# CHEBSB/PolarDecoding

Measured on AMD Instinct MI355X. Metric: decoded frames/sec, N=1024 K=512 CA-SCL L=8, higher is better.
Workload: dtype f64

## Files before the change

polardecoding_amd/csrc/scl_fast2.h:

```cpp
#pragma once
#include "octet_bits.h"
#include "scl_fast.h"

namespace polar {

template <typename R>
struct Fast2Cfg {
    static constexpr int NLOG = 10, N = 1024, NW = 32, TOP = 9, HI = 8, L = 8;
    static constexpr int NA = 32;
    static constexpr int WAVES = 4;
    static constexpr int MIN_WAVES_PER_SIMD = sizeof(R) == 8 ? 3 : 4;
    static constexpr int NFA = HI - 3;
    static constexpr size_t sc_l8 = 0;
    static constexpr size_t sc_l7 = sc_l8 + 8 * 256;
    static constexpr size_t sc_l6 = sc_l7 + 8 * 128;
    static constexpr size_t sc_tl = sc_l6 + 8 * 64;
    static constexpr size_t scratch_cw = sc_tl + 512;
    static constexpr size_t scratch_elems = 2 * scratch_cw;
    static constexpr size_t off_lut = 0;
    static constexpr size_t off_frz = off_lut + ((Lut<R>::bytes + 15) / 16) * 16;
    static constexpr size_t off_msk = off_frz + 4 * NW;
    static constexpr size_t off_kth = off_msk + 4 * CRC_MASK_ROWS * NW;
    static constexpr size_t off_stair = off_kth + 256 * 8;
    static constexpr size_t shared_bytes = off_stair + ((Stair<R>::bytes + 15) / 16) * 16;
    static constexpr size_t off_bl = 0;
    static constexpr size_t off_cw = off_bl + 4 * 2 * 8 * NW;
    static constexpr size_t off_cd = off_cw + 4 * 2 * 8 * NW;
    static constexpr size_t off_ky = off_cd + sizeof(R) * 32;
    static constexpr size_t off_sg = off_ky + 128;
    static constexpr size_t per_wave = off_sg + sizeof(R) * 512;
    static constexpr size_t total = shared_bytes + WAVES * per_wave;
};

template <int QP>
__device__ __forceinline__ double quadp(double x) { return quad_lanes<QP>(x); }
template <int QP>
__device__ __forceinline__ float quadp(float x) { return quad_lanes<QP>(x); }

template <bool FROM_Y>
struct Fast2Sigma { double sigma; };
template <>
struct Fast2Sigma<false> {};

template <typename R, typename IN, bool CRC_ON, bool FROM_Y>
struct Fast2Dec : Fast2Sigma<FROM_Y> {
    using C = Fast2Cfg<R>;
    static constexpr int N = C::N, NW = C::NW, TOP = C::TOP, HI = C::HI, L = 8, NFA = C::NFA;

    R A[C::NA];
    R a1;
    R bp_s, bp_d, bp_ts, bp_td;
    R PM;
    uint32_t ptr, bl0, fl;
    int logact;
    int p, c, pos, lane, gl;
    int own_addr, oth_addr;
    uint32_t pos0_mask;
    int cand_addr;
    Lut<R> lut;
    R *cand, *stg;
    uint32_t *blw, *curw, *keys;
    const unsigned char *kth;
    __amdgpu_buffer_rsrc_t rs_scr;
    __amdgpu_buffer_rsrc_t rs_in;
    unsigned cscr;
    unsigned csrc;
    static __device__ __forceinline__ __amdgpu_buffer_rsrc_t make_rsrc(const void *base, unsigned bytes)
    {
        return __builtin_amdgcn_make_buffer_rsrc(const_cast<void *>(base), 0, (int)bytes, 0x00020000);
    }
    typedef unsigned u2_t __attribute__((ext_vector_type(2)));
    static __device__ __forceinline__ double ld_buf(__amdgpu_buffer_rsrc_t r, unsigned eoff, double, int aux)
    {
        return aux ? __builtin_bit_cast(double, __builtin_amdgcn_raw_buffer_load_b64(r, eoff * 8u, 0, 16))
                   : __builtin_bit_cast(double, __builtin_amdgcn_raw_buffer_load_b64(r, eoff * 8u, 0, 0));
    }
    static __device__ __forceinline__ float ld_buf(__amdgpu_buffer_rsrc_t r, unsigned eoff, float, int aux)
    {
        return aux ? __builtin_bit_cast(float, __builtin_amdgcn_raw_buffer_load_b32(r, eoff * 4u, 0, 16))
                   : __builtin_bit_cast(float, __builtin_amdgcn_raw_buffer_load_b32(r, eoff * 4u, 0, 0));
    }
    static __device__ __forceinline__ void st_buf(__amdgpu_buffer_rsrc_t r, unsigned eoff, double v)
    {
        __builtin_amdgcn_raw_buffer_store_b64(__builtin_bit_cast(u2_t, v), r, eoff * 8u, 0, 0);
    }
    static __device__ __forceinline__ void st_buf(__amdgpu_buffer_rsrc_t r, unsigned eoff, float v)
    {
        __builtin_amdgcn_raw_buffer_store_b32(__builtin_bit_cast(unsigned, v), r, eoff * 4u, 0, 0);
    }
    struct SPtr {
        const Fast2Dec *d;
        unsigned off;
        struct Ref {
            const Fast2Dec *d;
            unsigned off;
            __device__ __forceinline__ void operator=(R v) const { st_buf(d->rs_scr, off, v); }
        };
        __device__ __forceinline__ SPtr operator+(int k) const { return SPtr{d, off + (unsigned)k}; }
        __device__ __forceinline__ Ref operator[](int k) const { return Ref{d, off + (unsigned)k}; }
    };
    static __device__ __forceinline__ R ld_sc(SPtr q) { return ld_buf(q.d->rs_scr, q.off, R(0), 1); }

    __device__ __forceinline__ int pa(int t) const { return (ptr >> (3 * (t - 4))) & 7; }
    __device__ __forceinline__ void set_pa(int t, int v) { ptr = (ptr & ~(7u << (3 * (t - 4)))) | ((uint32_t)v << (3 * (t - 4))); }
    __device__ __forceinline__ int pb(int t) const { return (ptr >> (3 * (NFA + t - 5))) & 7; }
    __device__ __forceinline__ void set_pb(int t, int v) { ptr = (ptr & ~(7u << (3 * (NFA + t - 5)))) | ((uint32_t)v << (3 * (NFA + t - 5))); }
    __device__ __forceinline__ R chk(R a, R b) const { return chk_lut1<R>(a, b, lut); }
    __device__ __forceinline__ R chks(R a, R b) const { return chk_lut1<R>(a, b, lut); }
    __device__ __forceinline__ R chv(int e) const
    {
        double v = (double)ld_buf(rs_in, csrc + (unsigned)e, IN(0), 0);
        if constexpr (FROM_Y) v = llr_from_y(v, this->sigma);
        return (R)v;
    }
    static __device__ __forceinline__ unsigned fresh(unsigned off)
    {
        __asm__ volatile("" : "+v"(off));
        return off;
    }
    __device__ __forceinline__ SPtr l8(int slot) const { return SPtr{this, fresh(cscr + (unsigned)(C::sc_l8 + slot * 256))}; }
    __device__ __forceinline__ SPtr l7(int slot) const { return SPtr{this, fresh(cscr + (unsigned)(C::sc_l7 + slot * 128))}; }
    __device__ __forceinline__ SPtr tls() const { return SPtr{this, fresh(cscr + (unsigned)C::sc_tl)}; }

    template <int T>
    __device__ __forceinline__ void f_reg()
    {
        constexpr int RO = (1 << T) / 4;
#pragma unroll
        for (int r = 0; r < RO; ++r) A[RO + r] = chk(A[2 * RO + r], A[3 * RO + r]);
        if constexpr (T >= 4) set_pa(T, p);
    }
    template <int T>
    __device__ __forceinline__ void g_reg()
    {
        constexpr int RO = (1 << T) / 4;
        const int sl = pa(T + 1) * 8 + gl;
        uint32_t w;
        if constexpr (T == 5) w = blw[pb(5) * NW + 1] >> pos;
        else w = bl0 >> (16 + pos);
#pragma unroll
        for (int r = 0; r < RO; ++r) {
            const R x = __shfl(A[2 * RO + r], sl), y = __shfl(A[3 * RO + r], sl);
            A[RO + r] = g_bit<R>(x, y, w, 4 * r);
        }
        set_pa(T, p);
    }
    __device__ __forceinline__ void g3()
    {
        const int sl = pa(4) * 8 + gl;
        const uint32_t w = bl0 >> (8 + pos);
#pragma unroll
        for (int r = 0; r < 2; ++r) {
            const R x = __shfl(A[4 + r], sl), y = __shfl(A[6 + r], sl);
            A[2 + r] = g_bit<R>(x, y, w, 4 * r);
        }
    }

    __device__ __forceinline__ void push_l6(R v)
    {
#pragma unroll
        for (int r = 16; r < 31; ++r) A[r] = A[r + 1];
        A[31] = v;
    }
    __device__ __forceinline__ void load_l6() { set_pa(6, p); }
    __device__ __forceinline__ R top_src(bool right, int idx, int q) const
    {
        const int seg = idx >> 4, within = idx & 15;
        const int e = 16 * q + within + 64 * (seg & 3) + 256 * (seg >> 2);
        return right ? chv(e) : ld_sc(tls() + e);
    }
    __device__ __forceinline__ void from_top(bool right, bool gstep)
    {
        vm_drain();
        const uint32_t *bt = blw + pb(TOP) * NW + 16;
        const uint32_t *bh = blw + pb(HI) * NW + 8;
        const SPtr o8 = l8(p), o7 = l7(p);
        const int w32 = (int)fresh((unsigned)(p * 4 + pos));
        const int nld = right ? 8 : 4;
        R *pre = A + 4;
#pragma unroll
        for (int m = 0; m < 8; ++m) pre[m] = (m < nld) ? top_src(right, w32 + 32 * m, 0) : R(0);
        for (int q = 0; q < 4; ++q) {
            lds_fence();
#pragma unroll
            for (int m = 0; m < 8; ++m)
                if (m < nld) stg[w32 + 32 * m] = pre[m];
            lds_fence();
            if (q < 3) {
#pragma unroll
                for (int m = 0; m < 8; ++m) pre[m] = (m < nld) ? top_src(right, w32 + 32 * m, q + 1) : R(0);
            }
#pragma unroll 1
            for (int i = 0; i < 4; ++i) {
                const int rr = 4 * q + i;
                const int e0 = pos + 4 * rr;
                const int sh = 4 * (rr & 7);
                const int wq = rr >> 3;
                const int wi = 4 * i + pos;
                R *v8 = A + 12;
#pragma unroll
                for (int k = 0; k < 4; ++k) {
                    const int e = e0 + 64 * k;
                    R x, y;
                    if (right) {
                        const uint32_t w0 = bt[2 * k + wq] >> pos, w1 = bt[8 + 2 * k + wq] >> pos;
                        x = g_bit<R>(stg[(k + 0) * 16 + wi], stg[(k + 8) * 16 + wi], w0, sh);
                        y = g_bit<R>(stg[(k + 4) * 16 + wi], stg[(k + 12) * 16 + wi], w1, sh);
                    } else {
                        x = stg[(k + 0) * 16 + wi];
                        y = stg[(k + 4) * 16 + wi];
                    }
                    if (gstep) v8[k] = g_bit<R>(x, y, bh[2 * k + wq] >> pos, sh);
                    else v8[k] = chk(x, y);
                    o8[e] = v8[k];
                }
                const R v70 = chk(v8[0], v8[2]), v71 = chk(v8[1], v8[3]);
                o7[e0] = v70;
                o7[e0 + 64] = v71;
                push_l6(chk(v70, v71));
            }
        }
        set_pa(8, p);
        set_pa(7, p);
        load_l6();
    }
    __device__ __forceinline__ void from_l8()
    {
        vm_drain();
        const SPtr s8 = l8(pa(8));
        const uint32_t *b7 = blw + pb(7) * NW + 4;
        const SPtr o7 = l7(p);
        constexpr int CP = sizeof(R) == 8 ? 2 : 4;
        for (int q = 0; q < 16 / CP; ++q) {
            R *in = A;
#pragma unroll
            for (int i = 0; i < CP; ++i) {
                const int e0 = pos + 4 * (CP * q + i);
#pragma unroll
                for (int k = 0; k < 4; ++k) in[4 * i + k] = ld_sc(s8 + e0 + 64 * k);
            }
#pragma unroll
            for (int i = 0; i < CP; ++i) {
                const int rr = CP * q + i;
                const int e0 = pos + 4 * rr;
                const int sh = 4 * (rr & 7);
                const int wq = rr >> 3;
                const R v70 = g_bit<R>(in[4 * i], in[4 * i + 2], b7[wq] >> pos, sh);
                const R v71 = g_bit<R>(in[4 * i + 1], in[4 * i + 3], b7[2 + wq] >> pos, sh);
                o7[e0] = v70;
                o7[e0 + 64] = v71;
                push_l6(chk(v70, v71));
            }
        }
        set_pa(7, p);
        load_l6();
    }
    __device__ __forceinline__ void from_l7()
    {
        vm_drain();
        const SPtr s7 = l7(pa(7)) + pos;
        const uint32_t *b6 = blw + pb(6) * NW + 2;
        const uint32_t w0 = b6[0] >> pos, w1 = b6[1] >> pos;
#pragma unroll
        for (int r = 0; r < 16; ++r) {
            const R x = ld_sc(s7 + 4 * r), y = ld_sc(s7 + 4 * r + 64);
            A[16 + r] = g_bit<R>(x, y, r < 8 ? w0 : w1, 4 * (r & 7));
        }
        set_pa(6, p);
    }

    __device__ __forceinline__ void octet_head(int o)
    {
        const int d = (o == 0) ? 10 : 3 + __builtin_ctz((unsigned)o);
        if (d >= 8) from_top(o >= N / 16, d == 8);
        else if (d == 7) from_l8();
        else if (d == 6) from_l7();
        else if (d == 5) g_reg<5>();
        else if (d == 4) g_reg<4>();
        else g3();
        if (d > 5) f_reg<5>();
        if (d > 4) f_reg<4>();
        if (d > 3) f_reg<3>();
    }
    __device__ __forceinline__ void octet_head_reg(int o)
    {
        const int d = 3 + __builtin_ctz((unsigned)o);
        if (d == 5) g_reg<5>();
        else if (d == 4) g_reg<4>();
        else g3();
        if (d > 4) f_reg<4>();
        if (d > 3) f_reg<3>();
    }

    template <int K>
    __device__ __forceinline__ void set_bit_k(int o, uint32_t bit)
    {
        if constexpr (K < 7) {
            bl0 |= bit << K;
        } else {
            const uint32_t c3 = octet_bits::level3((bl0 & 0x7Fu) | (bit << 7));
            bl0 &= ~0xFFu;
            set_bit7(o, c3);
        }
    }
    __device__ __forceinline__ void set_bit7(int o, uint32_t c3)
    {
        if ((o & 1) == 0) {
            bl0 = (bl0 & ~0xFF00u) | (c3 << 8);
            return;
        }
        const uint32_t c4 = (((bl0 >> 8) & 0xFFu) ^ c3) | (c3 << 8);
        if ((o & 2) == 0) {
            bl0 = (bl0 & 0xFFFFu) | (c4 << 16);
            return;
        }
        set_bit_lds(8 * o + 7, ((bl0 >> 16) ^ c4) | (c4 << 16));
    }
    __device__ __forceinline__ void set_bit_lds(int j, uint32_t cur)
    {
        const int row = (int)fresh((unsigned)(p * NW));
        lds_fence();
        if (pos == 0) curw[row] = cur;
        lds_fence();
        int t = 5;
        while (t < 10 && ((j >> t) & 1)) {
            const int nw = 1 << (t - 5);
            const int sb = pb(t);
            for (int w = pos; w < nw; w += 4) {
                const uint32_t cc = curw[row + w];
                const uint32_t l = blw[sb * NW + nw + w];
                curw[row + w] = l ^ cc;
                curw[row + w + nw] = cc;
            }
            lds_fence();
            ++t;
        }
        if (t < 10) {
            const int nw = 1 << (t - 5);
            for (int w = pos; w < nw; w += 4) blw[row + nw + w] = curw[row + w];
            set_pb(t, p);
            lds_fence();
        }
    }

    __device__ __forceinline__ uint32_t survivors(R c0, R c1)
    {
        lds_fence();
        if (pos == 0) {
            keys[2 * p] = metric_key(c0);
            keys[2 * p + 1] = metric_key(c1);
        }
        lds_fence();
        const unsigned char *kb = reinterpret_cast<const unsigned char *>(keys) - 64 * c;
        const uint32_t own = *reinterpret_cast<const uint32_t *>(kb + own_addr);
        const uint32_t oth = *reinterpret_cast<const uint32_t *>(kb + oth_addr);
        const uint32_t own1 = own + 1u;
        uint32_t acc = (oth - own1) >> 31;
        acc = __builtin_amdgcn_alignbit(acc, (uint32_t)dpp_i<0x121>((int)oth) - own1, 31);
        acc = __builtin_amdgcn_alignbit(acc, (uint32_t)dpp_i<0x122>((int)oth) - own1, 31);
        acc = __builtin_amdgcn_alignbit(acc, (uint32_t)dpp_i<0x123>((int)oth) - own1, 31);
        acc = __builtin_amdgcn_alignbit(acc, (uint32_t)dpp_i<0x124>((int)oth) - own1, 31);
        acc = __builtin_amdgcn_alignbit(acc, (uint32_t)dpp_i<0x125>((int)oth) - own1, 31);
        acc = __builtin_amdgcn_alignbit(acc, (uint32_t)dpp_i<0x126>((int)oth) - own1, 31);
        acc = __builtin_amdgcn_alignbit(acc, (uint32_t)dpp_i<0x127>((int)oth) - own1, 31);
        uint32_t cnt = __popc(acc);
        {
            auto r = __builtin_amdgcn_permlane16_swap(cnt, cnt, false, false);
            cnt = r[0] + r[1];
        }
        uint64_t b = __ballot(cnt <= (uint32_t)L);
        uint32_t m_a = (uint32_t)b & 0xFFFFu, m_b = (uint32_t)(b >> 32) & 0xFFFFu;
        if (sizeof(R) == 8 && (__popc(m_a) != L || __popc(m_b) != L)) {
            if (__popc(c ? m_b : m_a) != L) fl |= 0x4u;
            lds_fence();
            if (pos == 0) {
                cand[p] = c0;
                cand[8 + p] = c1;
            }
            lds_fence();
            const R *cb = reinterpret_cast<const R *>(reinterpret_cast<const unsigned char *>(cand) - (int)sizeof(R) * 16 * c);
            const R *mycand = reinterpret_cast<const R *>(reinterpret_cast<const unsigned char *>(cb) + cand_addr);
            const R mine = mycand[lane & 15];
            int n = 0;
#pragma unroll
            for (int m = 0; m < 16; ++m) n += (mycand[m] <= mine) ? 1 : 0;
            b = __ballot(n <= L);
            m_a = (uint32_t)b & 0xFFFFu;
            m_b = (uint32_t)(b >> 32) & 0xFFFFu;
        }
        return c ? m_b : m_a;
    }

    __device__ __forceinline__ bool trivial_prune(R cb, R cw) const
    {
        uint32_t mx = metric_key(cb) & pos0_mask;
        mx = max(mx, (uint32_t)dpp_i<0x128>((int)mx));
        {
            auto a = __builtin_amdgcn_permlane16_swap(mx, mx, false, false);
            mx = max(a[0], a[1]);
        }
        {
            auto a = __builtin_amdgcn_permlane32_swap(mx, mx, false, false);
            mx = max(a[0], a[1]);
        }
        return __ballot(mx >= (metric_key(cw) | ~pos0_mask)) == 0ull;
    }
    static __device__ __forceinline__ uint32_t sign_bit(double x) { return (uint32_t)__double2hiint(x) >> 31; }
    static __device__ __forceinline__ uint32_t sign_bit(float x) { return (uint32_t)__float_as_int(x) >> 31; }

    template <int K, bool FULL>
    __device__ __forceinline__ void decide(int o, bool frozen, R lam) { decide_t<K, FULL>(o, frozen, lam, lut.tabv(lam)); }
    template <int K, bool FULL>
    __device__ __forceinline__ void decide_t(int o, bool frozen, R lam, R tt)
    {
        if (frozen) {
            PM += tt + negmax(lam);
            set_bit_k<K>(o, 0u);
            return;
        }
        uint32_t bit;
        R pm;
        if (!FULL && logact < 3) {
            const R ph0 = tt + negmax(lam), ph1 = tt + posmax(lam);
            bit = (p >> logact) & 1;
            pm = PM + (bit ? ph1 : ph0);
            ++logact;
        } else {
            const uint32_t lneg = sign_bit(lam);
            const R cb = PM + tt, cw = PM + (tt + absr(lam));
            bit = (uint32_t)dpp_i<0x00>((int)lneg);
            pm = cb;
            if (!trivial_prune(cb, cw)) ranked<K>(lneg, cb, cw, bit, pm);
        }
        PM = pm;
        set_bit_k<K>(o, bit);
    }
    template <int K>
    __device__ __forceinline__ void ranked(uint32_t lneg, R cb, R cw, uint32_t &bit, R &pm)
    {
        const R c0 = lneg ? cw : cb, c1 = lneg ? cb : cw;
        const uint32_t mask = survivors(c0, c1);
        const uint32_t m0 = mask & 0xFFu, m1 = mask >> 8;
        const uint32_t m_both = m0 & m1, m_dead = ~(m0 | m1) & 0xFFu;
        if (__popc(mask) < L) fl |= 0x1u;
        const bool s0 = (m0 >> p) & 1, s1 = (m1 >> p) & 1;
        bit = (!s0 && s1) ? 1u : 0u;
        pm = bit ? c1 : c0;
        if (__ballot(m_dead != 0u) == 0ull) return;
        const bool dead = !s0 && !s1;
        const int myrank = __popc(m_dead & ((1u << p) - 1u));
        const bool refilled = dead && (myrank < __popc(m_both));
        const int src = (int)kth[m_both * 8 + myrank];
        const int sg = refilled ? src : p;
        const int sl = sg * 8 + gl;
        const R c1s = __shfl(c1, sl);
        ptr = __shfl(ptr, sl);
        bl0 = __shfl(bl0, sl);
        if constexpr ((K & 4) == 0) { A[2] = __shfl(A[2], sl); A[3] = __shfl(A[3], sl); }
        if constexpr ((K & 2) == 0) { A[1] = __shfl(A[1], sl); a1 = __shfl(a1, sl); }
        if constexpr ((K & 1) == 0) { bp_d = __shfl(bp_d, sl); bp_td = __shfl(bp_td, sl); }
        bit = refilled ? 1u : bit;
        pm = refilled ? c1s : pm;
    }

    __device__ __forceinline__ void frozen_prefix(int P, int nphi, bool regs, R &xl, R &yl)
    {
        const int w32 = p * 4 + pos, j0 = 8 * P;
        vm_drain();
        {
            const SPtr tl = tls();
            const SPtr o8 = l8(0), o7 = l7(0);
            R v8[8];
#pragma unroll
            for (int k = 0; k < 8; ++k) {
                const int e = w32 + 32 * k;
                v8[k] = chk(ld_sc(tl + e), ld_sc(tl + e + 256));
                o8[e] = v8[k];
            }
            lds_fence();
#pragma unroll
            for (int k = 0; k < 4; ++k) {
                const R v7 = chk(v8[k], v8[k + 4]);
                o7[w32 + 32 * k] = v7;
                stg[w32 + 32 * k] = v7;
            }
            set_pa(8, 0);
            set_pa(7, 0);
        }
        lds_fence();
#pragma unroll
        for (int t = 6; t >= 0; --t) {
            const int h = 1 << t;
            int idx[2];
            R x[2], y[2];
#pragma unroll
            for (int i = 0; i < 2; ++i) {
                const int b = w32 + 32 * i;
                idx[i] = ((b >> t) << (t + 1)) | (b & (h - 1));
                x[i] = stg[idx[i]];
                y[i] = stg[idx[i] + h];
            }
            if (t == 0) {
                xl = stg[126];
                yl = stg[127];
            }
            lds_fence();
#pragma unroll
            for (int i = 0; i < 2; ++i) {
                stg[idx[i]] = chk(x[i], y[i]);
                stg[idx[i] + h] = y[i] + x[i];
            }
            lds_fence();
            if (t >= 4 && regs) {
                const R *node = stg + ((j0 >> t) << t) + pos;
#pragma unroll
                for (int r = 0; r < h / 4; ++r) A[h / 4 + r] = node[4 * r];
            }
        }
#pragma unroll
        for (int k = 0; k < 4; ++k) {
            const R lam = stg[w32 + 32 * k];
            stg[128 + w32 + 32 * k] = lut.tabv(lam) + negmax(lam);
        }
        lds_fence();
        R pm = PM;
#pragma unroll 8
        for (int j = 0; j < nphi; ++j) pm += stg[128 + j];
        PM = pm;
        lds_fence();
    }

    __device__ __forceinline__ uint32_t fill_tail(uint32_t f2, R lam0, R xl, R yl)
    {
        uint32_t b0 = 0, b1 = 0;
        if (!(f2 & 1u)) {
            b0 = (p >> logact) & 1;
            ++logact;
        }
        PM += lut.tabv(lam0) + (b0 ? posmax(lam0) : negmax(lam0));
        const R lam1 = b0 ? -(xl - yl) : yl + xl;
        if (!(f2 & 2u)) {
            b1 = (p >> logact) & 1;
            ++logact;
        }
        PM += lut.tabv(lam1) + (b1 ? posmax(lam1) : negmax(lam1));
        return (b0 ? 0x55555555u : 0u) ^ (b1 ? 0xFFFFFFFFu : 0u);
    }
    __device__ __forceinline__ void fill_phase(int E, const uint32_t *frz, R xl, R yl)
    {
        const int w32 = (int)fresh((unsigned)(p * 4 + pos));
        const int qb = (p & 1) * 64;
        const uint32_t wv0 = fill_tail(frz[3] >> 30, stg[126], xl, yl);
        uint32_t wv1 = 0;
        lds_fence();
        blw[p * NW + 4 + pos] = wv0;
        lds_fence();
#pragma unroll 1
        for (int S = 128; S < E; S += 64) {
            vm_drain();
            const uint32_t wsel = S == 128 ? wv0 : wv1;
            uint32_t wq[2];
            wq[0] = (uint32_t)__shfl((int)wsel, gl) >> w32;
            wq[1] = (uint32_t)__shfl((int)wsel, 8 + gl) >> w32;
            if (S == 128) {
                const SPtr s8 = l8(0) + w32;
                R v8[8];
#pragma unroll
                for (int k = 0; k < 8; ++k) v8[k] = ld_sc(s8 + 32 * k);
#pragma unroll
                for (int q = 0; q < 2; ++q) {
                    const SPtr o7 = l7(q) + w32;
                    R v7[4];
#pragma unroll
                    for (int k = 0; k < 4; ++k) {
                        v7[k] = g_bit<R>(v8[k], v8[k + 4], wq[q], 0);
                        o7[32 * k] = v7[k];
                    }
                    stg[64 * q + w32] = chk(v7[0], v7[2]);
                    stg[64 * q + w32 + 32] = chk(v7[1], v7[3]);
                }
                set_pa(7, p & 1);
            } else {
#pragma unroll
                for (int q = 0; q < 2; ++q) {
                    const SPtr s7 = l7(q) + w32;
#pragma unroll
                    for (int i = 0; i < 2; ++i)
                        stg[64 * q + w32 + 32 * i] = g_bit<R>(ld_sc(s7 + 32 * i), ld_sc(s7 + 32 * i + 64), wq[q], 0);
                }
            }
            lds_fence();
#pragma unroll
            for (int t = 5; t >= 0; --t) {
                const int h = 1 << t;
                int idx[2];
                R x[2], y[2];
#pragma unroll
                for (int i = 0; i < 2; ++i) {
                    const int b = w32 + 32 * i;
                    idx[i] = ((b >> t) << (t + 1)) | (b & (h - 1));
                    x[i] = stg[idx[i]];
                    y[i] = stg[idx[i] + h];
                }
                if (t == 0) {
                    xl = stg[qb + 62];
                    yl = stg[qb + 63];
                }
                lds_fence();
#pragma unroll
                for (int i = 0; i < 2; ++i) {
                    stg[idx[i]] = chk(x[i], y[i]);
                    stg[idx[i] + h] = y[i] + x[i];
                }
                lds_fence();
            }
#pragma unroll
            for (int k = 0; k < 4; ++k) {
                const R lam = stg[w32 + 32 * k];
                stg[128 + w32 + 32 * k] = lut.tabv(lam) + negmax(lam);
            }
            lds_fence();
            R pm = PM;
#pragma unroll 2
            for (int j = 0; j < 62; ++j) pm += stg[128 + qb + j];
            PM = pm;
            const uint32_t wv = fill_tail(frz[(S + 62) >> 5] >> 30, stg[qb + 62], xl, yl);
            lds_fence();
            if (S == 128) {
                wv1 = wv;
                if (pos < 2) blw[p * NW + 2 + pos] = wv;
            } else {
                const uint32_t b = pos < 2 ? wv1 ^ wv : wv;
                blw[p * NW + 8 + pos] = wv0 ^ b;
                blw[p * NW + 12 + pos] = b;
            }
            lds_fence();
        }
    }

    template <bool FULL>
    __device__ __forceinline__ void octet_frozen_prefix(int o, bool last_frozen)
    {
        R xf = chks(A[2], A[3]), xg = A[3] + A[2];
        R yf = quadp<0x4E>(xf), yg = quadp<0x4E>(xg);
        {
            const R ff = chks(xf, yf), gf = xf + yf, fg = chks(xg, yg), gg = xg + yg;
            xf = (pos & 2) ? gf : ff;
            xg = (pos & 2) ? gg : fg;
        }
        yf = quadp<0xB1>(xf); yg = quadp<0xB1>(xg);
        R lf, lg;
        {
            const R ff = chks(xf, yf), gf = xf + yf, fg = chks(xg, yg), gg = xg + yg;
            lf = (pos & 1) ? gf : ff;
            lg = (pos & 1) ? gg : fg;
        }
        const R pf = lut.tabv(lf) + negmax(lf), pg = lut.tabv(lg) + negmax(lg);
        PM += pf;
        PM += quadp<0x55>(pf);
        PM += quadp<0xAA>(pf);
        PM += quadp<0xFF>(pf);
        PM += pg;
        PM += quadp<0x55>(pg);
        PM += quadp<0xAA>(pg);
        if (last_frozen) {
            PM += quadp<0xFF>(pg);
            set_bit7(o, 0u);
        } else {
            decide<7, FULL>(o, false, quadp<0xFF>(lg));
        }
    }

    struct ChkBp { R v, s, d, ts, td; };
    __device__ __forceinline__ ChkBp chk_bp(R x, R y) const
    {
        ChkBp r;
        r.s = x + y;
        r.d = x - y;
        r.ts = lut.tabv(r.s);
        r.td = lut.tabv(r.d);
        r.v = xor_sign(minabs(x, y), x, y) + (r.ts - r.td);
        return r;
    }
    static __device__ __forceinline__ R g_sel(R sum, R dif, uint32_t w, int sh)
    {
        const uint32_t m = (uint32_t)__builtin_amdgcn_sbfe((int)w, sh, 1);
        return Lut<R>::sel_mask(m, -dif, sum);
    }
    template <int K, bool FULL>
    __device__ __forceinline__ void leaf_pair(int o, uint32_t fm, R x1)
    {
        const ChkBp q = chk_bp(x1, quadp<0xB1>(x1));
        bp_d = q.d;
        bp_td = q.td;
        decide<K, FULL>(o, (fm >> K) & 1, q.v);
        const uint32_t m1 = (uint32_t)__builtin_amdgcn_sbfe((int)bl0, K, 1);
        decide_t<K + 1, FULL>(o, (fm >> (K + 1)) & 1, Lut<R>::sel_mask(m1, -bp_d, q.s), Lut<R>::sel_mask(m1, bp_td, q.ts));
    }
    template <bool FULL>
    __device__ __forceinline__ void octet(int o, uint32_t fm)
    {
        {
            const R s2 = A[2] + A[3], d2 = A[2] - A[3];
            const R v2 = xor_sign(minabs(A[2], A[3]), A[2], A[3]) + (lut.tabv(s2) - lut.tabv(d2));
            A[2] = s2;
            A[3] = d2;
            const R y2 = quadp<0x4E>(v2);
            const R s1 = v2 + y2, d1 = v2 - y2;
            const R v1 = xor_sign(minabs(v2, y2), v2, y2) + (lut.tabv(s1) - lut.tabv(d1));
            A[1] = s1;
            a1 = d1;
            leaf_pair<0, FULL>(o, fm, v1);
        }
        leaf_pair<2, FULL>(o, fm, g_sel(A[1], a1, octet_bits::level1_lo(bl0), pos));
        {
            const R v2 = g_sel(A[2], A[3], octet_bits::level2(bl0), pos);
            const R y2 = quadp<0x4E>(v2);
            const R s1 = v2 + y2, d1 = v2 - y2;
            const R v1 = xor_sign(minabs(v2, y2), v2, y2) + (lut.tabv(s1) - lut.tabv(d1));
            A[1] = s1;
            a1 = d1;
            leaf_pair<4, FULL>(o, fm, v1);
        }
        leaf_pair<6, FULL>(o, fm, g_sel(A[1], a1, octet_bits::level1_hi(bl0), pos));
    }
};

template <typename D, bool FULL>
__device__ __forceinline__ int octet_group(D &s, const uint32_t *frz, uint32_t &fword, int o)
{
    s.octet_head(o);
    for (;;) {
        if ((o & 3) == 0) fword = frz[o >> 2];
        const uint32_t fm = (fword >> (8 * (o & 3))) & 0xFFu;
        if ((fm & 0x7Fu) != 0x7Fu) s.template octet<FULL>(o, fm);
        else s.template octet_frozen_prefix<FULL>(o, fm == 0xFFu);
        ++o;
        if ((o & 7) == 0) break;
        s.octet_head_reg(o);
    }
    return o;
}

template <typename R, typename IN, bool CRC_ON, bool FROM_Y>
__device__ __forceinline__ void scl_fast2_body(const SclParams &P)
{
    using D = Fast2Dec<R, IN, CRC_ON, FROM_Y>;
    using C = Fast2Cfg<R>;
    constexpr int N = C::N, NW = C::NW, L = 8;
    extern __shared__ __attribute__((aligned(16))) unsigned char smem[];
    const int wave = __builtin_amdgcn_readfirstlane(threadIdx.x >> 6);
    unsigned char *base = smem + C::shared_bytes + (size_t)wave * C::per_wave;
    uint32_t *frz = reinterpret_cast<uint32_t *>(smem + C::off_frz);
    uint32_t *msk = reinterpret_cast<uint32_t *>(smem + C::off_msk);
    unsigned char *kth = smem + C::off_kth;

    Lut<R>::build(smem + C::off_lut, threadIdx.x, blockDim.x);
    for (int i = threadIdx.x; i < NW; i += blockDim.x) frz[i] = P.frozen[i];
    if (CRC_ON)
        for (int i = threadIdx.x; i < CRC_MASK_ROWS * NW; i += blockDim.x)
            msk[i] = P.crc_mask[(i & ~(NW - 1)) + ((i >> 3) & 3) + 4 * (i & 7)];
    for (int i = threadIdx.x; i < 256 * 8; i += blockDim.x) {
        int m = i >> 3, k = i & 7, idx = 0, seen = 0;
        for (int b = 0; b < 8; ++b)
            if ((m >> b) & 1) {
                if (seen == k) idx = b;
                ++seen;
            }
        kth[i] = (unsigned char)idx;
    }
    __syncthreads();

    D s;
    s.lane = threadIdx.x & 63;
    s.p = s.lane >> 3;
    s.c = (s.lane >> 2) & 1;
    s.pos = s.lane & 3;
    s.pos0_mask = s.pos == 0 ? 0xFFFFFFFFu : 0u;
    s.gl = s.lane & 7;
    s.lut.bind(smem + C::off_lut);
    s.kth = kth;
    s.blw = reinterpret_cast<uint32_t *>(base + C::off_bl) + s.c * 8 * NW;
    s.curw = reinterpret_cast<uint32_t *>(base + C::off_cw) + s.c * 8 * NW;
    s.cand = reinterpret_cast<R *>(base + C::off_cd) + s.c * 16;
    s.keys = reinterpret_cast<uint32_t *>(base + C::off_ky) + s.c * 16;
    s.stg = reinterpret_cast<R *>(base + C::off_sg) + s.c * 256;
    if constexpr (FROM_Y) s.sigma = P.sigma;
    {
        const int i = s.lane & 15, row = s.lane >> 4, cwr = row >> 1, h = row & 1;
        const int jj = (i + 8 * h) & 15;
        s.own_addr = 64 * cwr + 4 * (2 * (i & 7) + (i >> 3));
        s.oth_addr = 64 * cwr + 4 * (2 * (jj & 7) + (jj >> 3));
        s.cand_addr = (int)sizeof(R) * 16 * cwr;
    }
    const int lane = s.lane, p = s.p, c = s.c, pos = s.pos;
    const int wave_global = blockIdx.x * C::WAVES + wave;
    const int waves_total = gridDim.x * C::WAVES;
    R *scr_wave = reinterpret_cast<R *>(P.scratch) + (size_t)wave_global * C::scratch_elems;
    s.rs_scr = D::make_rsrc(scr_wave, (unsigned)(C::scratch_elems * sizeof(R)));
    s.cscr = (unsigned)c * (unsigned)C::scratch_cw;

    int lead = 0;
    while (lead < 15 && ((frz[lead >> 2] >> (8 * (lead & 3))) & 0xFFu) == 0xFFu) ++lead;
    lead = __builtin_amdgcn_readfirstlane(lead);
    const int E = P.fill_end;

    for (int pair = wave_global; 2 * pair < P.B;) {
        const int frame_raw = 2 * pair + c;
        const bool live = frame_raw < P.B;
        const int frame = live ? frame_raw : P.B - 1;
        s.rs_in = D::make_rsrc(reinterpret_cast<const IN *>(P.in) + (size_t)(2 * pair) * N, (unsigned)(2 * N * sizeof(IN)));
        s.csrc = (unsigned)(frame - 2 * pair) * (unsigned)N;
        {
            const auto t = s.tls();
            const int w = p * 4 + pos;
#pragma unroll 2
            for (int e = w; e < N / 2; e += 32) t[e] = s.chk(s.chv(e), s.chv(e + N / 2));
        }
        for (int w = lane; w < 2 * 8 * NW; w += 64) (s.blw - c * 8 * NW)[w] = 0;
        lds_fence();

        s.PM = R(0);
        s.ptr = 0;
        for (int t = 4; t <= 8; ++t) s.set_pa(t, p);
        for (int t = 5; t <= 9; ++t) s.set_pb(t, p);
        s.bl0 = 0;
        s.a1 = R(0);
#pragma unroll
        for (int r = 0; r < C::NA; ++r) s.A[r] = R(0);
        s.fl = 0;
        s.logact = 0;
        uint32_t fword = 0;

        int o_first = 0;
        if (E > 0 || lead > 0) {
            R xl, yl;
            s.frozen_prefix(E > 0 ? 15 : lead, E > 0 ? 126 : 8 * lead, E == 0, xl, yl);
            o_first = lead;
            if (E > 0) {
                s.fill_phase(E, frz, xl, yl);
                o_first = E >> 3;
            }
            fword = frz[o_first >> 2];
        }
        int o = o_first;
#pragma unroll 1
        while (o < N / 8 && s.logact < 3) o = octet_group<D, false>(s, frz, fword, o);
        while (o < N / 8) o = octet_group<D, true>(s, frz, fword, o);

        bool pass = false;
        if constexpr (CRC_ON) {
            lds_fence();
            uint32_t x[8];
#pragma unroll
            for (int j = 0; j < 8; ++j) x[j] = s.curw[p * NW + pos + 4 * j];
            typedef uint32_t u4_t __attribute__((ext_vector_type(4)));
            const u4_t *mk = reinterpret_cast<const u4_t *>(msk + 8 * pos);
            const int rows = (P.crc_r + 3) & ~3;
            uint32_t rem = 0;
#pragma unroll 1
            for (int i = 0; i < rows; i += 4) {
#pragma unroll
                for (int k = 0; k < 4; ++k) {
                    const u4_t a = mk[(i + k) * (NW / 4)], b = mk[(i + k) * (NW / 4) + 1];
                    const uint32_t acc = (x[0] & a.x) ^ (x[1] & a.y) ^ (x[2] & a.z) ^ (x[3] & a.w) ^ (x[4] & b.x) ^
                                         (x[5] & b.y) ^ (x[6] & b.z) ^ (x[7] & b.w);
                    rem |= (uint32_t)(__popc(acc) & 1) << (i + k);
                }
            }
            rem ^= (uint32_t)dpp_i<0xB1>((int)rem);
            rem ^= (uint32_t)dpp_i<0x4E>((int)rem);
            pass = rem == 0u;
        }
        const uint64_t bp_ = __ballot(pass && pos == 0);
        const uint64_t cwmask = 0x0101010101010101ull << (4 * c);
        const bool any = (bp_ & cwmask) != 0ull;
        int best = -1;
        R best_pm = R(0);
        for (int q = 0; q < L; ++q) {
            const R pq = __shfl(s.PM, q * 8 + 4 * c);
            const int okq = __shfl((int)(any ? pass : true), q * 8 + 4 * c);
            if (okq && (best < 0 || pq < best_pm)) {
                best = q;
                best_pm = pq;
            }
        }
        uint32_t fl = s.fl;
        if (any) fl |= 0x2u;
        lds_fence();
        {
            const int w = p * 4 + pos;
            uint32_t x = s.curw[best * NW + w];
            x ^= (x >> 1) & 0x55555555u;
            x ^= (x >> 2) & 0x33333333u;
            x ^= (x >> 4) & 0x0F0F0F0Fu;
            x ^= (x >> 8) & 0x00FF00FFu;
            x ^= (x >> 16) & 0x0000FFFFu;
#pragma unroll
            for (int hw = 1; hw < NW; hw <<= 1) {
                const int wo = w ^ hw;
                const uint32_t ov = __shfl(x, (wo >> 2) * 8 + 4 * c + (wo & 3));
                if (!(w & hw)) x ^= ov;
            }
            if (live) P.out_bits[(size_t)frame * NW + w] = x;
        }
        if (live && p == 0 && pos == 0) {
            if (P.pm) P.pm[frame] = (double)best_pm;
            if (P.flags) P.flags[frame] = fl;
        }
        lds_fence();
        pair = next_job_wave(P.queue, pair, waves_total, (P.B + 1) >> 1);
    }
}

template <typename R, typename IN, bool CRC_ON>
__global__ __launch_bounds__(256, (Fast2Cfg<R>::MIN_WAVES_PER_SIMD)) void k_scl_fast2(SclParams P)
{
    scl_fast2_body<R, IN, CRC_ON, false>(P);
}
template <typename R, typename IN, bool CRC_ON>
__global__ __launch_bounds__(256, (Fast2Cfg<R>::MIN_WAVES_PER_SIMD)) void k_scl_fast2_y(SclParams P)
{
    scl_fast2_body<R, IN, CRC_ON, true>(P);
}

}
```

Measured before the change: 15.11 million.

## Keep top-level LLRs in registers instead of reloading from scratch buffer

Input channel LLR loads are batched (issued all at once before a sched_barrier, then converted) and the top-level check results are held in the A register array. frozen_prefix and the first fill_phase step then read these registers rather than reloading the level-9, level-8 and level-7 values from global scratch, and two vm_drain waits are dropped. The aim is to cut scratch-buffer round trips and memory-latency stalls at the start of each frame. The cost is higher register pressure from reusing A slots and the larger batched load arrays, which could lower occupancy.

```diff
diff --git a/polardecoding_amd/csrc/scl_fast2.h b/polardecoding_amd/csrc/scl_fast2.h
--- a/polardecoding_amd/csrc/scl_fast2.h
+++ b/polardecoding_amd/csrc/scl_fast2.h
@@ -107,12 +107,14 @@
     __device__ __forceinline__ void set_pb(int t, int v) { ptr = (ptr & ~(7u << (3 * (NFA + t - 5)))) | ((uint32_t)v << (3 * (NFA + t - 5))); }
     __device__ __forceinline__ R chk(R a, R b) const { return chk_lut1<R>(a, b, lut); }
     __device__ __forceinline__ R chks(R a, R b) const { return chk_lut1<R>(a, b, lut); }
-    __device__ __forceinline__ R chv(int e) const
-    {
-        double v = (double)ld_buf(rs_in, csrc + (unsigned)e, IN(0), 0);
+    __device__ __forceinline__ IN chv_raw(int e) const { return ld_buf(rs_in, csrc + (unsigned)e, IN(0), 0); }
+    __device__ __forceinline__ R chv_cvt(IN raw) const
+    {
+        double v = (double)raw;
         if constexpr (FROM_Y) v = llr_from_y(v, this->sigma);
         return (R)v;
     }
+    __device__ __forceinline__ R chv(int e) const { return chv_cvt(chv_raw(e)); }
     static __device__ __forceinline__ unsigned fresh(unsigned off)
     {
         __asm__ volatile("" : "+v"(off));
@@ -466,15 +468,13 @@
     __device__ __forceinline__ void frozen_prefix(int P, int nphi, bool regs, R &xl, R &yl)
     {
         const int w32 = p * 4 + pos, j0 = 8 * P;
-        vm_drain();
         {
-            const SPtr tl = tls();
             const SPtr o8 = l8(0), o7 = l7(0);
-            R v8[8];
+            R *v8 = A + 16;
 #pragma unroll
             for (int k = 0; k < 8; ++k) {
                 const int e = w32 + 32 * k;
-                v8[k] = chk(ld_sc(tl + e), ld_sc(tl + e + 256));
+                v8[k] = chk(A[k], A[k + 8]);
                 o8[e] = v8[k];
             }
             lds_fence();
@@ -557,20 +557,16 @@
         lds_fence();
 #pragma unroll 1
         for (int S = 128; S < E; S += 64) {
-            vm_drain();
             const uint32_t wsel = S == 128 ? wv0 : wv1;
             uint32_t wq[2];
             wq[0] = (uint32_t)__shfl((int)wsel, gl) >> w32;
             wq[1] = (uint32_t)__shfl((int)wsel, 8 + gl) >> w32;
             if (S == 128) {
-                const SPtr s8 = l8(0) + w32;
-                R v8[8];
-#pragma unroll
-                for (int k = 0; k < 8; ++k) v8[k] = ld_sc(s8 + 32 * k);
+                const R *v8 = A + 16;
 #pragma unroll
                 for (int q = 0; q < 2; ++q) {
                     const SPtr o7 = l7(q) + w32;
-                    R v7[4];
+                    R *v7 = A + 4 * q;
 #pragma unroll
                     for (int k = 0; k < 4; ++k) {
                         v7[k] = g_bit<R>(v8[k], v8[k + 4], wq[q], 0);
@@ -582,12 +578,10 @@
                 set_pa(7, p & 1);
             } else {
 #pragma unroll
-                for (int q = 0; q < 2; ++q) {
-                    const SPtr s7 = l7(q) + w32;
+                for (int q = 0; q < 2; ++q)
 #pragma unroll
                     for (int i = 0; i < 2; ++i)
-                        stg[64 * q + w32 + 32 * i] = g_bit<R>(ld_sc(s7 + 32 * i), ld_sc(s7 + 32 * i + 64), wq[q], 0);
-                }
+                        stg[64 * q + w32 + 32 * i] = g_bit<R>(A[4 * q + i], A[4 * q + i + 2], wq[q], 0);
             }
             lds_fence();
 #pragma unroll
@@ -811,15 +805,6 @@
         const int frame = live ? frame_raw : P.B - 1;
         s.rs_in = D::make_rsrc(reinterpret_cast<const IN *>(P.in) + (size_t)(2 * pair) * N, (unsigned)(2 * N * sizeof(IN)));
         s.csrc = (unsigned)(frame - 2 * pair) * (unsigned)N;
-        {
-            const auto t = s.tls();
-            const int w = p * 4 + pos;
-#pragma unroll 2
-            for (int e = w; e < N / 2; e += 32) t[e] = s.chk(s.chv(e), s.chv(e + N / 2));
-        }
-        for (int w = lane; w < 2 * 8 * NW; w += 64) (s.blw - c * 8 * NW)[w] = 0;
-        lds_fence();
-
         s.PM = R(0);
         s.ptr = 0;
         for (int t = 4; t <= 8; ++t) s.set_pa(t, p);
@@ -827,10 +812,32 @@
         s.bl0 = 0;
         s.a1 = R(0);
 #pragma unroll
-        for (int r = 0; r < C::NA; ++r) s.A[r] = R(0);
+        for (int r = 16; r < C::NA; ++r) s.A[r] = R(0);
         s.fl = 0;
         s.logact = 0;
         uint32_t fword = 0;
+        {
+            constexpr int RB = sizeof(R) == 8 ? 16 : 8;
+            const auto t = s.tls();
+            const int w = p * 4 + pos;
+#pragma unroll
+            for (int b = 0; b < 16; b += RB) {
+                IN lo[RB], hi[RB];
+#pragma unroll
+                for (int k = 0; k < RB; ++k) {
+                    lo[k] = s.chv_raw(w + 32 * (b + k));
+                    hi[k] = s.chv_raw(w + 32 * (b + k) + N / 2);
+                }
+                __builtin_amdgcn_sched_barrier(0);
+#pragma unroll
+                for (int k = 0; k < RB; ++k) {
+                    s.A[b + k] = s.chk(s.chv_cvt(lo[k]), s.chv_cvt(hi[k]));
+                    t[w + 32 * (b + k)] = s.A[b + k];
+                }
+            }
+        }
+        for (int w = lane; w < 2 * 8 * NW; w += 64) (s.blw - c * 8 * NW)[w] = 0;
+        lds_fence();
 
         int o_first = 0;
         if (E > 0 || lead > 0) {
```

Result: no change. 15.24 million, median of 6 (+0.8%).
